# Meeso1/nmmo

Hardware: AMD Instinct MI355X
Metric: agent-steps/sec (whole node), 128-agent envs at 1/2/4/8 MI355X (higher is better)
Workload: dtype int16

## Files before the change

__graft_entry__.py:

```python

import os
import sys

ROOT = os.path.dirname(os.path.abspath(__file__))
if ROOT not in sys.path:
    sys.path.insert(0, ROOT)


def build() -> None:
    from nmmo_amd import build as nb

    nb.build(verbose=True)
    nb.build_heads(verbose=True)
    nb.build_ppo(verbose=True)
    nb.build_lstm(verbose=True)
    from oracle import oracle

    oracle.build(force=True)
    import nmmo_amd
    from nmmo_amd import _native

    _native.lib()
    from nmmo_amd import heads

    heads.lib()
    from nmmo_amd import ppo

    ppo.lib()
    from nmmo_amd import lstm

    lstm.lib()


def smoke() -> None:
    import numpy as np
    import torch

    from nmmo_amd.config import Config
    from nmmo_amd.engine import NmmoEngine
    from oracle.oracle import OracleEnvs

    assert torch.cuda.is_available(), "smoke() needs cuda:0"
    torch.cuda.set_device(0)
    cfg = Config.preset("C4", MAP_N=4, early_stop_agent_num=8)
    eng = NmmoEngine(cfg, 2, seed=3)
# ... 20 lines not shown
```

nmmo_amd/build.py:

```python

from __future__ import annotations

import concurrent.futures
import functools
import hashlib
import os
import subprocess
import sys
import tempfile
from typing import NamedTuple

HERE = os.path.dirname(os.path.abspath(__file__))
CSRC = os.path.join(HERE, "csrc")
INCLUDE = os.path.join(HERE, "..", "include")
LIB_DIR = os.path.join(HERE, "lib")
ARCH = os.environ.get("NMMO_OFFLOAD_ARCH", "gfx950")


class Lib(NamedTuple):
    file: str
    sources: list
    headers: list
    include: list
    link: list = []


LIBS = {
    "hip": Lib("libnmmo_hip.so",
               ["mapgen.hip", "tick.hip", "obs.hip", "wrap.hip", "storage.hip", "wire.hip", "wire_obs.hip",
                "native_obs.hip", "flat_obs.hip", "p2p.hip", "capi.hip"],
               ["agent_obs.h", "common.h", "host_api.h", "kernels.h", "obs_layout.h", "wire.h"], ["nmmo_hip.h"],
               ["-ldl"]),
    "heads": Lib("libnmmo_heads.so", ["heads.hip", "tile_enc.hip", "item_enc.hip"], ["common.h", "host_api.h"],
                 ["nmmo_hip.h", "nmmo_heads.h"]),
    "ppo": Lib("libnmmo_ppo.so", ["ppo.hip"], ["host_api.h"], ["nmmo_ppo.h"]),
    "lstm": Lib("libnmmo_lstm.so", ["lstm.hip"], ["host_api.h"], ["nmmo_lstm.h"]),
}
SOURCES, HEADERS = LIBS["hip"].sources, LIBS["hip"].headers
LIB_PATH = os.path.join(LIB_DIR, LIBS["hip"].file)
STAMPS_PATH = os.path.join(LIB_DIR, "libnmmo_hip_stamps.so")
FLAGS = [
    f"--offload-arch={ARCH}", "-O3", "-std=c++17", "-fPIC", "-fvisibility=hidden", "-Wall", "-Werror",
    "-ffp-contract=off",
]


def _hipcc() -> str:
    for cand in (os.environ.get("HIPCC"), "/opt/rocm/bin/hipcc", "hipcc"):
        if cand and (os.path.sep not in cand or os.path.exists(cand)):
            return cand
    raise RuntimeError("hipcc not found")


def lib_path(name: str = "hip") -> str:
    return os.path.join(LIB_DIR, LIBS[name].file)


def source_hash(name: str = "hip") -> str:
    row = LIBS[name]
    h = hashlib.sha256()
    for f in [os.path.join(CSRC, f) for f in row.sources + row.headers] + [
            os.path.join(INCLUDE, f) for f in row.include]:
        with open(f, "rb") as fh:
            h.update(os.path.basename(f).encode() + b"\0" + fh.read())
    return h.hexdigest()[:16]


def stale(name: str = "hip") -> bool:
    if not os.path.exists(lib_path(name)):
        return True
    with open(lib_path(name), "rb") as fh:
        return ("src=" + source_hash(name)).encode() not in fh.read()


def build_lib(name: str, force: bool = False, verbose: bool = False, stamps: bool = False) -> str:
    row = LIBS[name]
    if stamps and name != "hip":
        raise ValueError("only the product library has a stamps variant")
    out = STAMPS_PATH if stamps else lib_path(name)
    if not force and not stamps and not stale(name):
        return out
    os.makedirs(LIB_DIR, exist_ok=True)
    tmp = out + ".tmp"
    flags = [*FLAGS, *(["-DNMMO_STAMPS"] if stamps else []), f'-DNMMO_SRC_HASH="{source_hash(name)}"']
    with tempfile.TemporaryDirectory(prefix="nmmo_build_") as d:
        objs = [os.path.join(d, f + ".o") for f in row.sources]
        cmds = [[_hipcc(), *flags, "-c", os.path.join(CSRC, f), "-o", o] for f, o in zip(row.sources, objs)]
        if verbose:
            print("\n".join(" ".join(c) for c in cmds), file=sys.stderr)
        jobs = max(1, min(len(cmds), os.cpu_count() or 1, int(os.environ.get("MAX_JOBS", "8"))))
        with concurrent.futures.ThreadPoolExecutor(jobs) as ex:
            for f in [ex.submit(subprocess.check_call, c) for c in cmds]:
                f.result()
        subprocess.check_call([_hipcc(), f"--offload-arch={ARCH}", "-shared", "-fPIC", *objs, *row.link, "-o", tmp])
    os.replace(tmp, out)
    return out


build = functools.partial(build_lib, "hip")
build_heads = functools.partial(build_lib, "heads")
build_ppo = functools.partial(build_lib, "ppo")
build_lstm = functools.partial(build_lib, "lstm")


if __name__ == "__main__":
    for lib_name in LIBS:
        print(build_lib(lib_name, force="--force" in sys.argv, verbose=True))
```

nmmo_amd/csrc/agent_obs.h:

```cpp
#pragma once

#include <utility>

#include "kernels.h"
#include "wire.h"

namespace nmmo {

#ifndef NMMO_AO_WAVES
#define NMMO_AO_WAVES 4
#define NMMO_AO_AGENTS 16
#endif
constexpr int kAoWaves = NMMO_AO_WAVES;
constexpr int kAoAgents = NMMO_AO_AGENTS;
constexpr int kAoRows = kMaxSlots / 64;
constexpr uint32_t kAoEmpty = 0xFFFFFFFFu;
static_assert(kSize <= 256 && kMaxSlots <= 2 * 256 && kMaxSlots % 64 == 0, "packed entity word; two slots per thread (>= 256 threads)");
__host__ __device__ constexpr int ao_stride(int S) { return ((S + 1) >> 1 | 1) << 1; }
__host__ __device__ constexpr size_t ao_columns_lds(int S) {
  return ((size_t)NMMO_N_ENTITY_COLS * ao_stride(S) * 2 + 15) & ~(size_t)15;
}
constexpr size_t kAoPkBytes = (size_t)(kMaxSlots + 64) * 4;
__host__ __device__ constexpr size_t ao_entity_lds(int S) { return ao_columns_lds(S) + kAoPkBytes; }
__host__ __device__ inline uint32_t ao_pack(int slot, int row, int col, bool immune, bool danger, bool player) {
// ... 212 lines not shown
    const uint64_t b = __ballot(in);
    const int pos = nvis + __popcll(b & lanes_below());
    if (in && pos < kNObs) visw[pos] = x;
    nvis += __popcll(b);
  }
  return nvis;
}

__device__ __forceinline__ void ao_window_offsets(int (&mo)[2]) {
  mo[0] = mo[1] = 0;
#pragma unroll
  for (int i = 0; i < 4; i++) {
    const int t = lane_id() + 64 * i;
    const int o = t < 225 ? (t / 15 - kVision) * kSize + t % 15 - kVision : 0;
    mo[i >> 1] |= (o & 0xFFFF) << (16 * (i & 1));
  }
}
__device__ __forceinline__ int ao_window_off(const int (&mo)[2], int i) {
  return (int)(int16_t)(uint16_t)((uint32_t)mo[i >> 1] >> (16 * (i & 1)));
}

static_assert(F_ALCHEMY_LEVEL == F_MELEE_LEVEL + 14 && F_FISHING_LEVEL == F_MELEE_LEVEL + 6 &&
                  F_HERBALISM_LEVEL == F_MELEE_LEVEL + 8, "skill level fields");
__host__ __device__ constexpr uint64_t ao_req_lut() {
  uint64_t m = 0;
  for (int t = 0; t < 16; t++) {
    const int k = (t >= T_SPEAR && t <= T_WAND) ? t - T_SPEAR : (t >= T_WHETSTONE && t <= T_RUNES) ? t - T_WHETSTONE
                  : (t >= T_ROD && t <= T_CHISEL) ? 3 + t - T_ROD : 8;
    m |= (uint64_t)k << (4 * t);
  }
  return m;
}
static_assert(T_RATION == 16 && T_POTION == 17, "requirement table: ration -> fishing, potion -> herbalism");
__device__ __forceinline__ uint64_t ao_usable_ballot(const int16_t* T, int Sp, int ti, uint2 it, bool have) {
  const int lane = ao_lane();
  int lv = 0;
  if (lane < 8) {
    lv = T[(F_MELEE_LEVEL + 2 * lane) * Sp + ti];
  } else if (lane == 8) {
    lv = max((int)T[F_MELEE_LEVEL * Sp + ti], max((int)T[F_RANGE_LEVEL * Sp + ti], (int)T[F_MAGE_LEVEL * Sp + ti]));
  }
  const int type = it_type(it);
  const int k = type < 16 ? (int)((ao_req_lut() >> (4 * type)) & 15u) : type == T_RATION ? 3 : type == T_POTION ? 4 : 8;
  const int req = __shfl(lv, k);
  const bool eq = type >= T_HAT && type <= T_RUNES && it_equipped(it);
  return __ballot(have && !it_price(it) && (eq || it_level(it) <= req));
}

struct AoSections {
  uint64_t s0, s1[2], s3, s4, s5[2], s6[2], s7[2], s8, s9, s10[2], s11;
};
struct AoAgent {
  int a, ti, r, c, gold, aid, nv, ninv, prev_price;
  uint32_t mv;
};
template <bool kWrap>
__device__ __forceinline__ AoSections ao_sections(const ObsParams& p, const int16_t* T, int Sp, const uint32_t* visw,
                                                 const AoAgent& g, uint2 it) {
  const bool combat = (p.systems & NMMO_SYS_COMBAT) != 0;
  const bool item = (p.systems & NMMO_SYS_ITEM) != 0;
  const bool exch = item && (p.systems & NMMO_SYS_EXCHANGE) != 0;
  const bool no_give = kWrap && (p.wflags & kWrapObsNoGive);
  const bool no_danger = kWrap && (p.wflags & kWrapObsNoDangerous);
  const int lane = ao_lane();
  AoSections x;
  x.s1[0] = x.s1[1] = x.s5[0] = x.s5[1] = x.s7[0] = x.s7[1] = 0ull;
#pragma unroll
  for (int h = 0; h < 2; h++) {
    if (64 * h >= g.nv) break;
    const int k = 64 * h + lane;
    bool tgt = false, st = false;
    if (k < g.nv) {
      const uint32_t w = visw[k];
      const int q = ao_slot(w);
      tgt = combat && q != g.a && linf(g.r, g.c, ao_row(w), ao_col(w)) <= 3 && !ao_immune(w) &&
            !(no_danger && ao_danger(w));
      st = ao_player(w) && q != g.a && ao_row(w) == g.r && ao_col(w) == g.c;
    }
    x.s1[h] = __ballot(tgt);
    const uint64_t sb = __ballot(st);
    if (item && !no_give) x.s5[h] = sb;
    if (exch && !no_give) x.s7[h] = sb;
  }
  x.s1[1] |= 1ull << (kNObs - 64);
  x.s5[1] |= 1ull << (kNObs - 64);
  x.s7[1] |= 1ull << (kNObs - 64);
  const bool have = lane < g.ninv;
  const bool fr = have && !it_equipped(it) && !it_price(it);
  const uint64_t bfr = __ballot(fr);
  x.s3 = (item ? bfr : 0ull) | 1ull << kInv;
  x.s4 = (item && !no_give ? bfr : 0ull) | 1ull << kInv;
  x.s9 = (exch ? __ballot(have && !it_equipped(it)) : 0ull) | 1ull << kInv;
  x.s11 = (item ? ao_usable_ballot(T, Sp, g.ti, it, have) : 0ull) | 1ull << kInv;
  x.s0 = combat ? low_bits(kSecN[0]) : 0ull;
  x.s6[0] = x.s6[1] = x.s10[0] = x.s10[1] = 0ull;
  if (exch) {
    const int ng = no_give ? min(g.gold, 1) : min(g.gold, kSecN[6]);
    x.s6[0] = low_bits(ng);
    x.s6[1] = low_bits(ng - 64);
    x.s10[0] = low_bits(kSecN[10]);
    x.s10[1] = low_bits(kSecN[10] - 64);
    if constexpr (kWrap) {
      const int pp = g.prev_price;
      if ((p.wflags & kWrapObsPrice) && pp >= 0 && pp < kSecN[10]) {
        const uint64_t clr = ~(1ull << (pp & 63));
        if (pp < 64) x.s10[0] &= clr;
        else x.s10[1] &= clr;
      }
    }
  }
// ... 25 lines not shown
```

nmmo_amd/csrc/capi.hip:

```cpp
#include <math.h>
#include <stdlib.h>
#include <string.h>

#include <algorithm>
#include <map>
#include <mutex>
#include <vector>

#include "host_api.h"
#include "kernels.h"
#include "wire.h"

using namespace nmmo;

#define HIP_TRY(expr)                                                                    \
  do {                                                                                   \
    hipError_t _e = (expr);                                                              \
    if (_e != hipSuccess) return fail(NMMO_E_HIP, "%s: %s", #expr, hipGetErrorString(_e)); \
  } while (0)

struct NmmoHandle {
  NmmoConfig cfg;
  NmmoLayout layout;
  DevState st;
// ... 537 lines not shown
  if (fr && fr[0] == '1') HIP_TRY(hipMemAddressFree(ptr, a.bytes));
  return NMMO_OK;
}

int nmmo_set_step_records(NmmoHandle* h, uint8_t* dev_records, int32_t* dev_fault) {
  if (!h) return fail(NMMO_E_INVALID, "null handle");
  if (dev_records && h->cfg.obs_layout != NMMO_OBS_WIRE)
    return fail(NMMO_E_INVALID, "nmmo_set_step_records: step records come with the wire obs layout");
  if (dev_fault && !dev_records) return fail(NMMO_E_INVALID, "nmmo_set_step_records: dev_fault without records");
  h->d_recs = dev_records;
  h->d_recs_fault = dev_fault;
  return NMMO_OK;
}

int nmmo_obs_bind(NmmoHandle* h, const void* obs) {
  if (!h) return fail(NMMO_E_INVALID, "null handle");
  if (!h->d_zrow) return obs ? fail(NMMO_E_INVALID, "nmmo_obs_bind: flat or native obs layouts only") : NMMO_OK;
  HIP_TRY(hipSetDevice(h->device));
  HIP_TRY(hipDeviceSynchronize());
  HIP_TRY(hipMemset(h->d_zrow, 0, (size_t)h->st.n_envs * h->st.P * 8));
  h->zbuf = obs;
  h->ztag = obs ? h->ztag + 1 : h->ztag;
  return NMMO_OK;
}

int nmmo_obs_invalidate(NmmoHandle* h, void* stream) {
  if (!h) return fail(NMMO_E_INVALID, "null handle");
  if (!h->d_zrow) return NMMO_OK;
  HIP_TRY(hipSetDevice(h->device));
  HIP_TRY(hipMemsetAsync(h->d_zrow, 0, (size_t)h->st.n_envs * h->st.P * 8, (hipStream_t)stream));
  return NMMO_OK;
}

__global__ void obs_forget_envs_kernel(uint64_t* zrow, const int32_t* ids, int n_ids, int n_envs, int P) {
  const int i = blockIdx.x, e = ids[i];
  if ((unsigned)e >= (unsigned)n_envs) return;
  for (int a = threadIdx.x; a < P; a += blockDim.x) zrow[(size_t)e * P + a] = 0;
}

int nmmo_obs_invalidate_envs(NmmoHandle* h, const int32_t* env_ids, int32_t n_ids, void* stream) {
  if (!h) return fail(NMMO_E_INVALID, "null handle");
  if (n_ids < 0 || n_ids > h->st.n_envs) return fail(NMMO_E_INVALID, "n_ids %d not in 0..%d", n_ids, h->st.n_envs);
  if (n_ids > 0 && !env_ids) return fail(NMMO_E_INVALID, "null env_ids");
  if (!h->d_zrow || n_ids == 0) return NMMO_OK;
  HIP_TRY(hipSetDevice(h->device));
  hipLaunchKernelGGL(obs_forget_envs_kernel, dim3(n_ids), dim3(128), 0, (hipStream_t)stream, h->d_zrow, env_ids,
                     n_ids, h->st.n_envs, h->st.P);
  HIP_TRY(hipGetLastError());
  return NMMO_OK;
}

__global__ void obs_forget_tile_kernel(uint64_t* zst, const int32_t* ids, int n_envs, int P) {
  const int e = ids ? ids[blockIdx.x] : (int)blockIdx.x;
  if ((unsigned)e >= (unsigned)n_envs) return;
  for (int a = threadIdx.x; a < P; a += blockDim.x) zst[(size_t)e * P + a] |= kZsTile;
}

int nmmo_obs_invalidate_sections(NmmoHandle* h, const int32_t* env_ids, int32_t n_ids, uint32_t sections,
                                 void* stream) {
  if (!h) return fail(NMMO_E_INVALID, "null handle");
  if (!env_ids) n_ids = h->st.n_envs;
  if (n_ids < 0 || n_ids > h->st.n_envs) return fail(NMMO_E_INVALID, "n_ids %d not in 0..%d", n_ids, h->st.n_envs);
  if (!h->d_zrow || n_ids == 0 || sections == 0) return NMMO_OK;
  HIP_TRY(hipSetDevice(h->device));
  const bool tile_only = sections == NMMO_OBS_SEC_TILE && h->cfg.obs_layout == NMMO_OBS_FLAT;
  if (!tile_only) {
// ... 682 lines not shown
```

nmmo_amd/csrc/flat_obs.hip:

```cpp
#include "agent_obs.h"

namespace nmmo {

#ifndef NMMO_FO_ABL
#define NMMO_FO_ABL 0
#endif
#ifndef NMMO_FO_STAMPS
#define NMMO_FO_STAMPS 0
#endif
#if NMMO_FO_STAMPS
constexpr int kFoStamps = 12;
__device__ uint64_t fo_stamp_buf[1 << 17][kFoStamps];
__device__ uint64_t fo_wave_buf[1 << 15][6];
#define FO_STAMP(k) fst[k] = __builtin_amdgcn_s_memtime()
#else
#define FO_STAMP(k) (void)0
#endif
#ifndef NMMO_FO_XCD
#define NMMO_FO_XCD 1
#endif
#ifndef NMMO_FO_TILE_SKIP
#define NMMO_FO_TILE_SKIP 0
#endif
#ifndef NMMO_FO_TASK_BATCH
// ... 86 lines not shown
  return (uint64_t)(uint32_t)__builtin_amdgcn_readlane((int)g.lo, g.j10 + slot) |
         (uint64_t)(uint32_t)__builtin_amdgcn_readlane((int)g.hi, g.j10 + slot) << 32;
}
template <int kC>
__device__ __forceinline__ void fo_put(float* row, FoImg& g, uint64_t m, float aid, float tick) {
  constexpr int sl = fo_slot(kC);
  const int lane = ao_lane();
  const bool same = g.ext && m == fo_prev(g, sl);
  if constexpr (kC == kFoChunks - 1) {
    constexpr int n = kMaskN - 64 * kC;
    if (!same) {
      if (lane < n + 2) fo_st(row, 64 * kC + lane, lane < n ? fo_bit(m) : lane == n ? aid : tick);
      g.nst += n + 2;
    } else {
      if (lane == n + 1) fo_st(row, 64 * kC + lane, tick);
      g.nst += 1;
    }
  } else if (!same) {
    fo_st(row, 64 * kC + lane, fo_bit(m));
    g.nst += 64;
  }
  g.nimg = writelane<2 * sl>((int)(uint32_t)m, g.nimg);
  g.nimg = writelane<2 * sl + 1>((int)(uint32_t)(m >> 32), g.nimg);
}
template <int kC>
__device__ __forceinline__ void fo_tail_chunks(float* row, FoImg& g, const AoSections& x, uint64_t buy17, float aid,
                                               float tick) {
  if constexpr (kC < kFoChunks) {
    uint64_t m = fo_chunk<kC>(x);
    if constexpr (kC == kFoTail0) m |= buy17 | 1ull << ((kWireBuyLo + NMMO_MARKET_ROWS) & 63);
    fo_put<kC>(row, g, m, aid, tick);
    fo_tail_chunks<kC + 1>(row, g, x, buy17, aid, tick);
  }
}

struct IcDesc {
  uint32_t tmA, tmB;
  uint32_t f;
};
__device__ __forceinline__ IcDesc ic_desc(int col) {
  auto bits = [](int lo, int hi) { return ((2u << hi) - 1u) & ~((1u << lo) - 1u); };
  IcDesc d{0u, 0u, 0u};
  auto bf = [&](int sel, int sh, int wd) { d.f = (uint32_t)(sel | sh << 1 | wd << 6); };
  switch (col) {
    case 0: bf(1, 16, 16); break;
    case 1: bf(0, 0, 5); break;
    case 2: d.f = 1u << 11; break;
    case 3: bf(0, 5, 4); break;
    case 5: bf(1, 0, 16); break;
    case 6: case 7: case 8:
      d.tmA = 1u << (T_SPEAR + col - 6) | 1u << (T_WHETSTONE + col - 6);
      d.f = 5u << 12 | 5u << 20;
      break;
    case 9: case 10: case 11:
      d.tmA = bits(T_HAT, T_BOTTOM);
      d.tmB = bits(T_ROD, T_CHISEL);
      d.f = 3u << 12 | 2u << 16;
      break;
    case 12: d.tmA = 1u << T_POTION; d.f = 5u << 12 | 50u << 20; break;
    case 13: d.tmA = 1u << T_RATION; d.f = 5u << 12 | 50u << 20; break;
    case 14: bf(0, 9, 1); break;
    case 15: bf(0, 10, 7); break;
    default: break;
  }
  return d;
}
// ... 162 lines not shown
  const int nm = min(max(sg.nm, 0), NMMO_MARKET_ROWS), nst = fo_staged(nm);
  const uint2 lwd = ao_listing_load(p, e, sg);
  auto listings = [&]() {
    if constexpr (kMirror) {
      uint4* gd = reinterpret_cast<uint4*>(gat) + w * kGatIt * 64 + lane;
      gd[0] = gq0;
      if constexpr (kGatIt > 1) gd[64] = gq1;
      if constexpr (kGatIt > 2) gd[128] = gq2;
      if constexpr (kGatIt > 3) gd[192] = gq3;
    }
    if (tid < nm) {
      mpo[tid] = (uint16_t)(it_price(lwd) | ((sg.mv >> 16) & 255) << 8);
      if (tid < nst) mtop[-tid] = lwd;
    }
    for (int j = tid + (int)blockDim.x; j < nm; j += blockDim.x) {
      const int v = p.mlist[(size_t)e * NMMO_MARKET_ROWS + j];
      const int own = (v >> 16) & 255, slot = (v >> 24) & 15;
      const uint2 wd = p.items[((size_t)e * P + own) * kInv + slot];
      mpo[j] = (uint16_t)(it_price(wd) | own << 8);
      if (j < nst) mtop[-j] = wd;
    }
  };
  if constexpr (kMirror)
    ao_stage_windows_at<kAoAgents, kFoWinRowBytes / 4, true>(p, e, g, wpr, wpc, wst, ist, listings);
  else
    ao_stage_windows<kAoAgents, kFoWinRowBytes / 4>(p, e, g, T, Sp, wst, ist, listings, []() { __syncthreads(); });
#if NMMO_FO_STAMPS
  wst_[2] = __builtin_amdgcn_s_memtime();
#endif
  asm volatile("" : "+v"(img.x), "+v"(img.y), "+v"(pinv.x), "+v"(pinv.y), "+v"(my_prev));
  if (!img_ok) img = make_uint2(0u, 0u);
  if (!pinv_ok) pinv = make_uint2(0u, 0u);
  const int my_h = !zvl ? (kNObs | NMMO_MARKET_ROWS << 12) : zzl ? 0 : (zs_hv(my_s) | zs_hm(my_s) << 12);
  int nrows = 0;
  unsigned long long nbytes = 0;
  int wo[2];
  ao_win_offsets<kFoWinRowBytes>(wo);
  int toff[4];
#pragma unroll
  for (int i = 0; i < 4; i++) {
    const int t = lane + 64 * i;
    toff[i] = ((t / 15 - kVision) & 255) | (t % 15 - kVision) * 256;
  }
  const int ef = lane & 31, eh = lane >> 5;
  const int iq = lane >> 4;
  const IcDesc icd = ic_desc(lane & 15);

#if NMMO_FO_STAMPS
  wst_[3] = __builtin_amdgcn_s_memtime();
#endif
#pragma unroll 1
  for (int j = 0; j < ((NMMO_FO_ABL & 64) ? 0 : kPerWave); j++) {
    const int a = abase + kAoWaves * j;
    if (a >= P) break;
    const int lane = ao_lane();
    FoArgs kp = (FoArgs)__builtin_amdgcn_kernarg_segment_ptr();
    asm volatile("" : "+s"(kp));
    auto grow = (__attribute__((address_space(1))) float*)(p.obs + ((NMMO_FO_ABL & 256)
        ? (size_t)(((e * P + a) & 15) + 16 * (blockIdx.x & 7)) : (size_t)e * P + a) * elems);
    asm volatile("" : "+s"(grow));
    float* row = (float*)grow;
    const bool zv = (zvalid >> j) & 1;
    const int hj = __builtin_amdgcn_readlane(my_h, j);
    const int hv = hj & 4095, hm = hj >> 12;
    if (!__builtin_amdgcn_readlane(my_alive, j)) {
      if ((zzero >> j) & 1) {
// ... 8 lines not shown
      if (zv) {
        wave_zero(row, 0, kFlatEntity + hv * NMMO_N_ENTITY_COLS);
        wave_zero(row, kFlatInv, kFlatMarket + hm * 16);
        wave_zero(row, kFlatTask, elems);
        nbytes += 4ull * (kFlatEntity + hv * NMMO_N_ENTITY_COLS + kFlatMarket + hm * 16 - kFlatInv + elems - kFlatTask);
      } else {
        wave_zero(row, 0, elems);
        nbytes += 4ull * elems;
      }
      if (lane == 0) {
        kp->zrow[(size_t)e * P + a] = kp->ztag;
        kp->zst[(size_t)e * P + a] = kZsZero;
      }
      nrows++;
      continue;
    }
    nrows++;
#if NMMO_FO_STAMPS
    uint64_t fst[kFoStamps];
#endif
    FO_STAMP(0);
    const int la = a - g * kAoAgents;
    const int rcj = __builtin_amdgcn_readlane((int)my_rc, j);
    const int r = (int16_t)(rcj & 0xFFFF), c = rcj >> 16;
    const int16_t* Ta = kMirror ? T + la * kMirrorCols : T;
    const int Spa = kMirror ? 1 : Sp, tia = kMirror ? 0 : a;
    if constexpr (kMirror) visw = visw_all + (w * kPerWave + j) * kFoVisw;
    const int gold = __builtin_amdgcn_readfirstlane(Ta[F_GOLD * Spa + tia]);
    const int aid = __builtin_amdgcn_readfirstlane(Ta[F_ID * Spa + tia]);
    const uint8_t* wa = wsb + la * kFoWinAgentBytes;
    uint32_t wm[4];
#pragma unroll
    for (int i = 0; i < 4; i++) wm[i] = lane + 64 * i < 225 ? wa[ao_win_off(wo, i)] : 0u;
    const uint2 it = lane < kInv ? ist[la * kInv + lane] : make_uint2(0u, 0u);
    const uint32_t mv = ao_move_bits(wm[1]);
    const int ninv = __builtin_ctzll(~__ballot(lane < kInv && it_type(it) != 0));
    int nv;
    if constexpr (kMirror) {
      nv = __builtin_amdgcn_readlane(my_nv, j);
    } else {
      nv = (NMMO_FO_ABL & 32) ? 0 : min(fo_compact(pr, r, c, visw), kNObs);
      __builtin_amdgcn_fence(__ATOMIC_RELEASE, "wavefront");
      __builtin_amdgcn_wave_barrier();
      __builtin_amdgcn_fence(__ATOMIC_ACQUIRE, "wavefront");
    }

    FO_STAMP(1);
    const bool ext = (zextv >> j) & 1;
    FoImg fg{ext, img.x, img.y, 10 * j, 0, 0};
    if (!(NMMO_FO_ABL & 1)) {
      AoAgent ag;
      ag.a = a;
      ag.ti = tia;
      ag.r = r;
      ag.c = c;
      ag.gold = gold;
      ag.aid = aid;
      ag.nv = nv;
      ag.ninv = ninv;
      ag.prev_price = kWrap ? __builtin_amdgcn_readlane(my_prev, j) : -1;
      ag.mv = mv;
      const AoSections x = ao_sections<kWrap>(p, Ta, Spa, visw, ag, it);
      FO_STAMP(2);
      fg.ext = ext;
      fo_put<0>(row, fg, fo_chunk<0>(x), 0.f, 0.f);
      auto buy_word = [&](int m) {
        const int k = 64 * m + lane;
        bool bv = false;
        if (exch && k < nm) {
          const uint32_t po = mpo[k];
          bv = (int)(po & 255u) <= gold && (int)(po >> 8) != a;
        }
        return __ballot(bv);
      };
      const int nbuy = max(nm, hm);
      const int clast = max(1, min((kWireBuyLo + nbuy - 1) >> 6, 16));
      uint64_t bprev = nm > 0 ? buy_word(0) : 0ull;
      fo_put<1>(row, fg, fo_chunk<1>(x) | bprev << (kWireBuyLo & 63), 0.f, 0.f);
      FO_STAMP(3);
#pragma unroll 1
      for (int cc = 2; cc <= clast; cc++) {
        const uint64_t bcur = 64 * (cc - 1) < nm ? buy_word(cc - 1) : 0ull;
        fo_st(row, 64 * cc + lane, fo_bit(bcur << (kWireBuyLo & 63) | bprev >> (64 - (kWireBuyLo & 63))));
// ... 18 lines not shown
        if (ef < NMMO_N_ENTITY_COLS) {
          float v = 0.f;
          if (k < nv) {
            const uint32_t vw = visw[k];
            const int tv = kMirror ? gj[k * kMirrorCols + ef] : T[ef * Sp + ao_slot(vw)];
            v = (float)(epos ? (int)((vw >> esh) & 255u) : tv);
          }
          fo_st(row, de + k0 * NMMO_N_ENTITY_COLS, v);
        }
      }
      if constexpr (kMirror) {
        if (nv2 > kFoGather) {
          const int16_t* Mk = kp->frows + (size_t)e * kMaxSlots * kMirrorCols;
#pragma unroll 1
          for (int k0 = kFoGather; k0 < nv2; k0 += 2) {
            const int k = k0 + eh;
            if (ef < NMMO_N_ENTITY_COLS) {
              float v = 0.f;
              if (k < nv) {
                const uint32_t vw = visw[k];
                const int tv = Mk[(size_t)min(ao_slot(vw), kMaxSlots - 1) * kMirrorCols + ef];
                v = (float)(epos ? (int)((vw >> esh) & 255u) : tv);
              }
              fo_st(row, de + k0 * NMMO_N_ENTITY_COLS, v);
            }
          }
        }
      }
      const int hz = max(nv2, hv);
      wave_zero(row, kFlatEntity + nv2 * NMMO_N_ENTITY_COLS, kFlatEntity + hz * NMMO_N_ENTITY_COLS);
      nbytes += 4ull * (hz * NMMO_N_ENTITY_COLS + max(nm, hm) * 16);
    }
    FO_STAMP(6);
    const int jl = (12 * j + lane) & 63;
    const uint32_t px = (uint32_t)__shfl((int)pinv.x, jl), py = (uint32_t)__shfl((int)pinv.y, jl);
    const bool inv_same = ext && __ballot(lane < kInv && (px != it.x || py != it.y)) == 0ull;
    if (!inv_same) {
#pragma unroll
      for (int h = 0; h < ((NMMO_FO_ABL & 4) ? 0 : kInv * 16 / 64); h++) {
        const int q = 4 * h + iq;
        float v = 0.f;
        if (4 * h < ninv && q < ninv) v = ic_value(ist[la * kInv + q], aid, icd);
        fo_st(row, kFlatInv + 64 * h + lane, v);
      }
      nbytes += 4ull * kInv * 16;
    }
    FO_STAMP(7);
    const int nms = (NMMO_FO_ABL & 8) ? 0 : fo_staged(nm);
    for (int k = lane; k < nms * 16; k += 64) fo_st(row, kFlatMarket + k, ic_value(mtop[-(k >> 4)], (mpo[k >> 4] >> 8) + 1, icd));
    if (nm > nms && !(NMMO_FO_ABL & 8)) {
      for (int k = nms * 16 + lane; k < nm * 16; k += 64) {
        const int q = k >> 4;
        const int v = kp->mlist[(size_t)e * NMMO_MARKET_ROWS + q];
        const uint2 wd = kp->items[((size_t)e * P + ((v >> 16) & 255)) * kInv + ((v >> 24) & 15)];
        fo_st(row, kFlatMarket + k, ic_value(wd, (mpo[q] >> 8) + 1, icd));
      }
    }
    wave_zero(row, kFlatMarket + nm * 16, kFlatMarket + max(nm, hm) * 16);
    FO_STAMP(8);
    const int task = __builtin_amdgcn_readlane(my_task, j);
    if (!((ztask >> j) & 1)) {
      const float* temb = kp->task + (size_t)task * tdim;
      int k0 = 0;
      for (; k0 + kFoTaskBatch * 64 <= tdim; k0 += kFoTaskBatch * 64) {
        float t[kFoTaskBatch];
#pragma unroll
        for (int i = 0; i < kFoTaskBatch; i++) t[i] = temb[k0 + 64 * i + lane];
#pragma unroll
        for (int i = 0; i < kFoTaskBatch; i++) fo_st(row, kFlatTask + k0 + 64 * i + lane, t[i]);
      }
      for (int k = k0 + lane; k < tdim; k += 64) fo_st(row, kFlatTask + k, temb[k]);
      nbytes += 4ull * tdim;
    }
    FO_STAMP(9);
    const uint32_t ppos = (uint32_t)__builtin_amdgcn_readlane((int)img.x, 40 + j);
    const bool tkn = NMMO_FO_TILE_SKIP && ext && !((ztile >> j) & 1);
    const bool same_r = tkn && (int)(ppos & 255u) == r, same_c = tkn && (int)((ppos >> 8) & 255u) == c;
    if (!(NMMO_FO_ABL & 16)) {
      float* dt = row + kFlatTask + tdim + 3 * lane;
#pragma unroll
      for (int i = 0; i < 4; i++) {
        if (lane + 64 * i < 225) {
          const float vr = (float)(r + ((toff[i] << 24) >> 24)), vc = (float)(c + (toff[i] >> 8)), vm = (float)wm[i];
          if (NMMO_FO_TILE_SKIP) {
            if (!same_r) dt[192 * i] = vr;
            if (!same_c) dt[192 * i + 1] = vc;
            dt[192 * i + 2] = vm;
          } else {
            typedef float f3 __attribute__((ext_vector_type(3)));
            const f3 v = {vr, vc, vm};
            __builtin_memcpy(dt + 192 * i, &v, 12);
          }
        }
      }
      nbytes += 4ull * 225 * (1 + !same_r + !same_c);
    }
    FO_STAMP(10);
    {
      uint32_t* zx = reinterpret_cast<uint32_t*>(kp->zext + ((size_t)e * P + a) * kZext);
      int wv = fg.nimg;
      if (lane == 20) wv = r | c << 8;
      if (lane == 21) wv = 0;
      if (lane < 22) zx[lane] = (uint32_t)wv;
      if (!inv_same && lane < kInv) reinterpret_cast<uint2*>(zx + 22)[lane] = it;
      if (lane == 0) {
        if (!zv) kp->zrow[(size_t)e * P + a] = kp->ztag;
        kp->zst[(size_t)e * P + a] = zs_pack(nv2, nm, task) | kZsExt;
      }
    }
#if NMMO_FO_STAMPS
    FO_STAMP(11);
    if (lane == 0 && (size_t)e * P + a < (1u << 17))
      for (int k = 0; k < kFoStamps; k++) fo_stamp_buf[(size_t)e * P + a][k] = fst[k];
#endif
    if constexpr (!kMirror) {
      __builtin_amdgcn_fence(__ATOMIC_RELEASE, "wavefront");
      __builtin_amdgcn_wave_barrier();
      __builtin_amdgcn_fence(__ATOMIC_ACQUIRE, "wavefront");
    }
  }
#if NMMO_FO_STAMPS
  wst_[4] = __builtin_amdgcn_s_memtime();
  wst_[5] = (uint64_t)e | (uint64_t)nrows << 32;
  {
    const size_t wi = ((size_t)blockIdx.y * gridDim.x + blockIdx.x) * kAoWaves + w;
    if (lane == 0 && wi < (1u << 15))
      for (int k = 0; k < 6; k++) fo_wave_buf[wi][k] = wst_[k];
  }
#endif
  if (p.rows_out && lane == 0 && nrows) {
    atomicAdd(&p.rows_out[2 * e], (unsigned long long)nrows);
// ... 52 lines not shown
```

nmmo_amd/engine.py:

```python

from __future__ import annotations

import ctypes

import numpy as np
import torch

from . import abi
from ._native import NativeError, check, layout, lib


class TickFault(NativeError):

    def __init__(self, word: int, where: str = ""):
        self.word = int(word)
        self.code, self.env = self.word & 0xFF, self.word >> 8
        what = abi.FAULT_NAMES.get(self.code, f"code {self.code}")
        super().__init__(f"{where + ': ' if where else ''}tick fault word {self.word:#x}: {what} "
                         f"(env / list position {self.env})")


class NmmoEngine:
    def __init__(self, config, n_envs: int, seed: int = 0, device=None, task_embedding=None,
                 env_index_base: int = 0):
# ... 197 lines not shown
    def set_step_records(self, records, fault=None):
        if records is not None and (records.dtype != torch.uint8 or records.device != self.device
                                    or not records.is_contiguous() or records.numel() < 8 * self.n_envs * self.P):
            raise ValueError("records must be a contiguous uint8 tensor of >= 8 * n_envs * P bytes on the "
                             "engine's device")
        if fault is not None and (fault.dtype != torch.int32 or fault.device != self.device):
            raise ValueError("fault must be an int32 tensor on the engine's device")
        self._step_records = (records, fault)
        check(lib().nmmo_set_step_records(self.h, None if records is None else ctypes.c_void_p(records.data_ptr()),
                                          None if fault is None else ctypes.c_void_p(fault.data_ptr())),
              "nmmo_set_step_records")

    def obs_invalidate(self):
        check(lib().nmmo_obs_invalidate(self.h, self._stream()), "nmmo_obs_invalidate")

    def obs_invalidate_envs(self, env_ids):
        if env_ids.dtype != torch.int32 or env_ids.device != self.device or not env_ids.is_contiguous():
            raise ValueError("env_ids must be a contiguous int32 tensor on the engine's device")
        with torch.cuda.device(self.device):
            check(lib().nmmo_obs_invalidate_envs(self.h, self._ptr(env_ids), env_ids.numel(), self._stream()),
                  "nmmo_obs_invalidate_envs")
        self._inv_ids = env_ids

    def obs_invalidate_sections(self, sections: int, env_ids=None):
        if env_ids is not None and (env_ids.dtype != torch.int32 or env_ids.device != self.device
                                    or not env_ids.is_contiguous()):
            raise ValueError("env_ids must be a contiguous int32 tensor on the engine's device")
        with torch.cuda.device(self.device):
            check(lib().nmmo_obs_invalidate_sections(self.h, None if env_ids is None else self._ptr(env_ids),
                                                     0 if env_ids is None else env_ids.numel(), int(sections),
                                                     self._stream()), "nmmo_obs_invalidate_sections")
        self._inv_ids = env_ids

    def get_fault(self) -> int:
        f = ctypes.c_int32()
        check(lib().nmmo_get_fault(self.h, ctypes.byref(f)), "nmmo_get_fault")
        return f.value

    def check_fault(self, where: str = ""):
        f = self.get_fault()
        if f:
            raise TickFault(f, where)

    def fault_into(self, dst):
        with torch.cuda.device(self.device):
            check(lib().nmmo_fault_into(self.h, self._ptr(dst), self._stream()), "nmmo_fault_into")

    def inject_fault(self, word: int):
        check(lib().nmmo_inject_fault(self.h, int(word)), "nmmo_inject_fault")

    def read_timing(self):
        ms = (ctypes.c_double * 3)()
        n = ctypes.c_int32()
        check(lib().nmmo_read_timing(self.h, ms, ctypes.byref(n)), "nmmo_read_timing")
        return ms[0], ms[1], n.value, ms[2]

    def get_state(self) -> np.ndarray:
        n = self.layout.state_bytes_per_env * self.n_envs
        buf = np.zeros(n, np.uint8)
        check(lib().nmmo_get_state(self.h, buf.ctypes.data_as(ctypes.c_void_p), n), "nmmo_get_state")
        return buf

    def set_state(self, buf: np.ndarray):
        buf = np.ascontiguousarray(buf, dtype=np.uint8)
        check(lib().nmmo_set_state(self.h, buf.ctypes.data_as(ctypes.c_void_p), buf.nbytes),
              "nmmo_set_state")
# ... 55 lines not shown
```

Measured before the change: 328.1 million.

## Batch action-mask computation across a wave's agents in mirror flat-obs path

Adds a per-wave mask pass that computes the action-mask chunks, buy-order ballots, inventory diffs and zext row state for all agents in a wave at once, using 16-lane groups per agent instead of a full wave per agent. The per-agent loop then only stores the chunks that changed, read from the precomputed words, and skips its own inventory, move and zext bookkeeping in the mirror path. It also adds a test-hook library build and a debug API to read obs row state. This aims to cut the serial per-agent ballot and shuffle work and redundant loads, at the cost of more register pressure and more complex logic.

New measurement: 342.5 million, median of 6. 1.04x the previous value.

```diff
diff --git a/__graft_entry__.py b/__graft_entry__.py
--- a/__graft_entry__.py
+++ b/__graft_entry__.py
@@ -11,6 +11,7 @@
     from nmmo_amd import build as nb
 
     nb.build(verbose=True)
+    nb.build_hooks(verbose=True)
     nb.build_heads(verbose=True)
     nb.build_ppo(verbose=True)
     nb.build_lstm(verbose=True)
diff --git a/nmmo_amd/build.py b/nmmo_amd/build.py
--- a/nmmo_amd/build.py
+++ b/nmmo_amd/build.py
@@ -39,6 +39,7 @@
 SOURCES, HEADERS = LIBS["hip"].sources, LIBS["hip"].headers
 LIB_PATH = os.path.join(LIB_DIR, LIBS["hip"].file)
 STAMPS_PATH = os.path.join(LIB_DIR, "libnmmo_hip_stamps.so")
+HOOKS_PATH = os.path.join(LIB_DIR, "libnmmo_hip_hooks.so")
 FLAGS = [
     f"--offload-arch={ARCH}", "-O3", "-std=c++17", "-fPIC", "-fvisibility=hidden", "-Wall", "-Werror",
     "-ffp-contract=off",
@@ -73,16 +74,25 @@
         return ("src=" + source_hash(name)).encode() not in fh.read()
 
 
-def build_lib(name: str, force: bool = False, verbose: bool = False, stamps: bool = False) -> str:
+def _embeds(path: str, name: str) -> bool:
+    if not os.path.exists(path):
+        return False
+    with open(path, "rb") as fh:
+        return ("src=" + source_hash(name)).encode() in fh.read()
+
+
+def build_lib(name: str, force: bool = False, verbose: bool = False, stamps: bool = False, hooks: bool = False) -> str:
     row = LIBS[name]
-    if stamps and name != "hip":
-        raise ValueError("only the product library has a stamps variant")
-    out = STAMPS_PATH if stamps else lib_path(name)
-    if not force and not stamps and not stale(name):
+    if (stamps or hooks) and name != "hip":
+        raise ValueError("only the product library has variants")
+    out = STAMPS_PATH if stamps else HOOKS_PATH if hooks else lib_path(name)
+    if not force and hooks and _embeds(out, name):
+        return out
+    if not force and not stamps and not hooks and not stale(name):
         return out
     os.makedirs(LIB_DIR, exist_ok=True)
     tmp = out + ".tmp"
-    flags = [*FLAGS, *(["-DNMMO_STAMPS"] if stamps else []), f'-DNMMO_SRC_HASH="{source_hash(name)}"']
+    flags = [*FLAGS, *(["-DNMMO_STAMPS"] if stamps else []), *(["-DNMMO_TEST_HOOKS"] if hooks else []), f'-DNMMO_SRC_HASH="{source_hash(name)}"']
     with tempfile.TemporaryDirectory(prefix="nmmo_build_") as d:
         objs = [os.path.join(d, f + ".o") for f in row.sources]
         cmds = [[_hipcc(), *flags, "-c", os.path.join(CSRC, f), "-o", o] for f, o in zip(row.sources, objs)]
@@ -98,6 +108,7 @@
 
 
 build = functools.partial(build_lib, "hip")
+build_hooks = functools.partial(build_lib, "hip", hooks=True)
 build_heads = functools.partial(build_lib, "heads")
 build_ppo = functools.partial(build_lib, "ppo")
 build_lstm = functools.partial(build_lib, "lstm")
@@ -106,3 +117,4 @@
 if __name__ == "__main__":
     for lib_name in LIBS:
         print(build_lib(lib_name, force="--force" in sys.argv, verbose=True))
+    print(build_hooks(force="--force" in sys.argv, verbose=True))
diff --git a/nmmo_amd/csrc/agent_obs.h b/nmmo_amd/csrc/agent_obs.h
--- a/nmmo_amd/csrc/agent_obs.h
+++ b/nmmo_amd/csrc/agent_obs.h
@@ -268,6 +268,14 @@
   return m;
 }
 static_assert(T_RATION == 16 && T_POTION == 17, "requirement table: ration -> fishing, potion -> herbalism");
+__device__ __forceinline__ int ao_req_lane(int type) {
+  return type < 16 ? (int)((ao_req_lut() >> (4 * type)) & 15u) : type == T_RATION ? 3 : type == T_POTION ? 4 : 8;
+}
+__device__ __forceinline__ bool ao_usable(uint2 it, bool have, int req) {
+  const int type = it_type(it);
+  const bool eq = type >= T_HAT && type <= T_RUNES && it_equipped(it);
+  return have && !it_price(it) && (eq || it_level(it) <= req);
+}
 __device__ __forceinline__ uint64_t ao_usable_ballot(const int16_t* T, int Sp, int ti, uint2 it, bool have) {
   const int lane = ao_lane();
   int lv = 0;
@@ -276,11 +284,15 @@
   } else if (lane == 8) {
     lv = max((int)T[F_MELEE_LEVEL * Sp + ti], max((int)T[F_RANGE_LEVEL * Sp + ti], (int)T[F_MAGE_LEVEL * Sp + ti]));
   }
-  const int type = it_type(it);
-  const int k = type < 16 ? (int)((ao_req_lut() >> (4 * type)) & 15u) : type == T_RATION ? 3 : type == T_POTION ? 4 : 8;
-  const int req = __shfl(lv, k);
-  const bool eq = type >= T_HAT && type <= T_RUNES && it_equipped(it);
-  return __ballot(have && !it_price(it) && (eq || it_level(it) <= req));
+  const int req = __shfl(lv, ao_req_lane(it_type(it)));
+  return __ballot(ao_usable(it, have, req));
+}
+
+__device__ __forceinline__ void ao_row_preds(uint32_t w, int a, int r, int c, bool combat, bool no_danger, bool& tgt,
+                                             bool& st) {
+  const int q = ao_slot(w);
+  tgt = combat && q != a && linf(r, c, ao_row(w), ao_col(w)) <= 3 && !ao_immune(w) && !(no_danger && ao_danger(w));
+  st = ao_player(w) && q != a && ao_row(w) == r && ao_col(w) == c;
 }
 
 struct AoSections {
@@ -307,11 +319,7 @@
     const int k = 64 * h + lane;
     bool tgt = false, st = false;
     if (k < g.nv) {
-      const uint32_t w = visw[k];
-      const int q = ao_slot(w);
-      tgt = combat && q != g.a && linf(g.r, g.c, ao_row(w), ao_col(w)) <= 3 && !ao_immune(w) &&
-            !(no_danger && ao_danger(w));
-      st = ao_player(w) && q != g.a && ao_row(w) == g.r && ao_col(w) == g.c;
+      ao_row_preds(visw[k], g.a, g.r, g.c, combat, no_danger, tgt, st);
     }
     x.s1[h] = __ballot(tgt);
     const uint64_t sb = __ballot(st);
diff --git a/nmmo_amd/csrc/capi.hip b/nmmo_amd/csrc/capi.hip
--- a/nmmo_amd/csrc/capi.hip
+++ b/nmmo_amd/csrc/capi.hip
@@ -593,6 +593,22 @@
   return NMMO_OK;
 }
 
+#ifdef NMMO_TEST_HOOKS
+__attribute__((visibility("default"))) int nmmo_debug_obs_row_state(NmmoHandle* h, uint64_t* tag, uint64_t* zrow,
+                                                                     uint64_t* zst, uint64_t* zext) {
+  if (!h || !tag || !zrow || !zst || !zext) return fail(NMMO_E_INVALID, "null argument");
+  if (!h->d_zrow || !h->d_zext) return fail(NMMO_E_INVALID, "nmmo_debug_obs_row_state: flat obs layout only");
+  const size_t rows = (size_t)h->st.n_envs * h->st.P;
+  HIP_TRY(hipSetDevice(h->device));
+  HIP_TRY(hipDeviceSynchronize());
+  HIP_TRY(hipMemcpy(zrow, h->d_zrow, rows * 8, hipMemcpyDeviceToHost));
+  HIP_TRY(hipMemcpy(zst, h->d_zrow + rows, rows * 8, hipMemcpyDeviceToHost));
+  HIP_TRY(hipMemcpy(zext, h->d_zext, rows * kZext * 8, hipMemcpyDeviceToHost));
+  *tag = h->zbuf ? h->ztag : 0;
+  return NMMO_OK;
+}
+#endif
+
 __global__ void obs_forget_envs_kernel(uint64_t* zrow, const int32_t* ids, int n_ids, int n_envs, int P) {
   const int i = blockIdx.x, e = ids[i];
   if ((unsigned)e >= (unsigned)n_envs) return;
diff --git a/nmmo_amd/csrc/flat_obs.hip b/nmmo_amd/csrc/flat_obs.hip
--- a/nmmo_amd/csrc/flat_obs.hip
+++ b/nmmo_amd/csrc/flat_obs.hip
@@ -142,6 +142,166 @@
     fo_put<kC>(row, g, m, aid, tick);
     fo_tail_chunks<kC + 1>(row, g, x, buy17, aid, tick);
   }
+}
+
+constexpr int kFoPassRows = 16;
+static_assert(kFoPassRows == 16 && kAoAgents / kAoWaves * kFoPassRows <= 64 && kInv <= kFoPassRows &&
+                  kFoGather <= kFoPassRows, "a 16-lane group per agent");
+constexpr int kFoBuyLane = 48;
+struct FoPass {
+  uint32_t lo, hi;
+  uint64_t chg;
+  uint64_t idiff;
+};
+template <int kSl>
+__device__ __forceinline__ void fo_pass_chunks(const AoSections& x, int sl, uint64_t& m) {
+  if constexpr (kSl < 10) {
+    constexpr int c = kSl < 2 ? kSl : kSl - 2 + kFoTail0;
+    static_assert(fo_slot(c) == kSl, "tracked chunk");
+    const uint64_t mc = fo_chunk<c>(x);
+    if (sl == kSl) m = mc;
+    fo_pass_chunks<kSl + 1>(x, sl, m);
+  }
+}
+template <bool kWrap>
+__device__ __forceinline__ FoPass fo_mask_pass(const ObsParams& p, int e, int w, int abase, int nm, const int16_t* own,
+                                               const uint32_t* visw, const uint8_t* wsb, const uint2* ist,
+                                               const uint16_t* mpo, int my_nv, uint32_t my_rc, int my_prev, int my_alive,
+                                               int my_task, uint64_t zvalid, uint64_t zextv, uint2 img, uint2 pinv) {
+  constexpr int kPerWave = kAoAgents / kAoWaves;
+  const bool combat = (p.systems & NMMO_SYS_COMBAT) != 0;
+  const bool item = (p.systems & NMMO_SYS_ITEM) != 0;
+  const bool exch = item && (p.systems & NMMO_SYS_EXCHANGE) != 0;
+  const bool no_give = kWrap && (p.wflags & kWrapObsNoGive);
+  const bool no_danger = kWrap && (p.wflags & kWrapObsNoDangerous);
+  const int lane = lane_id(), P = p.P;
+  const int gj = lane >> 4, gk = lane & 15, ga = abase + kAoWaves * gj, gla = w + kAoWaves * gj;
+  const int grc = __shfl((int)my_rc, gj);
+  const int gr = (int16_t)(grc & 0xFFFF), gc = grc >> 16;
+  bool tgt = false, st = false;
+  if (gk < __shfl(my_nv, gj)) ao_row_preds(visw[gj * kFoVisw + gk], ga, gr, gc, combat, no_danger, tgt, st);
+  const uint64_t tb = __ballot(tgt), sb = __ballot(st);
+  const uint2 it = gk < kInv ? ist[gla * kInv + gk] : make_uint2(0u, 0u);
+  const uint64_t occ = __ballot(gk < kInv && it_type(it) != 0);
+  const bool have = gk < __builtin_ctz(~((uint32_t)(occ >> (16 * gj)) & 0xFFFFu));
+  const uint64_t bfr = __ballot(have && !it_equipped(it) && !it_price(it));
+  const uint64_t bse = __ballot(have && !it_equipped(it));
+  uint64_t bus;
+  {
+    const int16_t* lvs = own + gla * kMirrorCols + F_MELEE_LEVEL;
+    int lv = 0;
+    if (gk < 8) lv = lvs[2 * gk];
+    else if (gk == 8) lv = max((int)lvs[0], max((int)lvs[F_RANGE_LEVEL - F_MELEE_LEVEL], (int)lvs[F_MAGE_LEVEL - F_MELEE_LEVEL]));
+    const int req = __shfl(lv, 16 * gj + ao_req_lane(it_type(it)));
+    bus = __ballot(ao_usable(it, have, req));
+  }
+  const int ja = min(lane / 10, kPerWave - 1), sl = lane - 10 * (lane / 10), la = w + kAoWaves * ja;
+  const uint64_t noop = 1ull << (kNObs - 64);
+  uint64_t t0 = (uint32_t)(tb >> (16 * ja)) & 0xFFFFu, t1 = 0ull, s0 = (uint32_t)(sb >> (16 * ja)) & 0xFFFFu, s1 = 0ull;
+#pragma unroll 1
+  for (int j = 0; j < kPerWave; j++) {
+    const int nv = __builtin_amdgcn_readlane(my_nv, j);
+    if (nv <= kFoPassRows) continue;
+    const int rcj = __builtin_amdgcn_readlane((int)my_rc, j), a = abase + kAoWaves * j;
+    const int r = (int16_t)(rcj & 0xFFFF), c = rcj >> 16;
+    uint64_t tj[2] = {0ull, 0ull}, sj[2] = {0ull, 0ull};
+#pragma unroll
+    for (int h = 0; h < 2; h++) {
+      if (64 * h >= nv) break;
+      const int k = 64 * h + lane;
+      bool tg = false, sm = false;
+      if (k < nv) ao_row_preds(visw[j * kFoVisw + k], a, r, c, combat, no_danger, tg, sm);
+      tj[h] = __ballot(tg);
+      sj[h] = __ballot(sm);
+    }
+    if (ja == j) t0 = tj[0], t1 = tj[1], s0 = sj[0], s1 = sj[1];
+  }
+  AoSections x;
+  x.s1[0] = t0;
+  x.s1[1] = t1 | noop;
+  x.s5[0] = item && !no_give ? s0 : 0ull;
+  x.s5[1] = (item && !no_give ? s1 : 0ull) | noop;
+  x.s7[0] = exch && !no_give ? s0 : 0ull;
+  x.s7[1] = (exch && !no_give ? s1 : 0ull) | noop;
+  const uint64_t ifr = (uint32_t)(bfr >> (16 * ja)) & 0xFFFFu;
+  x.s3 = (item ? ifr : 0ull) | 1ull << kInv;
+  x.s4 = (item && !no_give ? ifr : 0ull) | 1ull << kInv;
+  x.s9 = (exch ? (uint64_t)((uint32_t)(bse >> (16 * ja)) & 0xFFFFu) : 0ull) | 1ull << kInv;
+  x.s11 = (item ? (uint64_t)((uint32_t)(bus >> (16 * ja)) & 0xFFFFu) : 0ull) | 1ull << kInv;
+  x.s0 = combat ? low_bits(kSecN[0]) : 0ull;
+  x.s6[0] = x.s6[1] = x.s10[0] = x.s10[1] = 0ull;
+  if (exch) {
+    const int gold = own[la * kMirrorCols + F_GOLD];
+    const int ng = no_give ? min(gold, 1) : min(gold, kSecN[6]);
+    x.s6[0] = low_bits(ng);
+    x.s6[1] = low_bits(ng - 64);
+    x.s10[0] = low_bits(kSecN[10]);
+    x.s10[1] = low_bits(kSecN[10] - 64);
+    if constexpr (kWrap) {
+      const int pp = __shfl(my_prev, ja);
+      if ((p.wflags & kWrapObsPrice) && pp >= 0 && pp < kSecN[10]) {
+        const uint64_t clr = ~(1ull << (pp & 63));
+        if (pp < 64) x.s10[0] &= clr;
+        else x.s10[1] &= clr;
+      }
+    }
+  }
+  {
+    const uint8_t* wa = wsb + la * kFoWinAgentBytes;
+    uint32_t b = 0u;
+#pragma unroll
+    for (int d = 0; d < 5; d++)
+      if (!impassable((int)wa[(kVision + dir_dr(d)) * kFoWinRowBytes + kVision + dir_dc(d)])) b |= 1u << d;
+    x.s8 = b;
+  }
+  uint64_t m = 0ull;
+  fo_pass_chunks<0>(x, sl, m);
+  uint64_t bw0 = 0ull, bw15 = 0ull;
+  FoPass o;
+  o.lo = img.x;
+  o.hi = img.y;
+  if (exch && nm > 0) {
+    const uint32_t po0 = lane < nm ? mpo[lane] : 0u, po15 = 15 * 64 + lane < nm ? mpo[15 * 64 + lane] : 0u;
+#pragma unroll
+    for (int j = 0; j < kPerWave; j++) {
+      const int a = abase + kAoWaves * j;
+      const int gold = __builtin_amdgcn_readfirstlane((int)own[(w + kAoWaves * j) * kMirrorCols + F_GOLD]);
+      const uint64_t b0 = __ballot(lane < nm && (int)(po0 & 255u) <= gold && (int)(po0 >> 8) != a);
+      uint64_t b15 = 0ull;
+      if (nm > 15 * 64) b15 = __ballot(15 * 64 + lane < nm && (int)(po15 & 255u) <= gold && (int)(po15 >> 8) != a);
+      if (ja == j) bw0 = b0, bw15 = b15;
+      if (lane == kFoBuyLane + j) o.lo = (uint32_t)b0, o.hi = (uint32_t)(b0 >> 32);
+    }
+  }
+  if (sl == 1) m |= bw0 << (kWireBuyLo & 63);
+  if (sl == 2) m |= bw15 >> (64 - (kWireBuyLo & 63)) | 1ull << ((kWireBuyLo + NMMO_MARKET_ROWS) & 63);
+  const bool ext = (zextv >> ja) & 1;
+  o.chg = __ballot(lane < 10 * kPerWave && (!ext || (uint32_t)m != img.x || (uint32_t)(m >> 32) != img.y));
+  if (lane < 10 * kPerWave) o.lo = (uint32_t)m, o.hi = (uint32_t)(m >> 32);
+  const int ji = min(lane / kInv, kPerWave - 1);
+  const uint2 iw = ist[(w + kAoWaves * ji) * kInv + lane % kInv];
+  const bool idl = lane < kInv * kPerWave && (!((zextv >> ji) & 1) || iw.x != pinv.x || iw.y != pinv.y);
+  o.idiff = __ballot(idl);
+  {
+    const int jp = lane < 10 * kPerWave ? ja : min(lane - 10 * kPerWave, kPerWave - 1);
+    const size_t ai = (size_t)e * P + min(abase + kAoWaves * jp, P - 1);
+    uint2 wv = make_uint2(o.lo, o.hi);
+    const int rcp = __shfl((int)my_rc, jp);
+    if (lane >= 10 * kPerWave) {
+      wv = make_uint2((uint32_t)((int)(int16_t)(rcp & 0xFFFF) | (rcp >> 16) << 8), 0u);
+    }
+    const int alp = __shfl(my_alive, jp);
+    if (lane < 11 * kPerWave && alp) reinterpret_cast<uint2*>(p.zext)[ai * kZext + (lane < 10 * kPerWave ? sl : 10)] = wv;
+    const size_t ii = (size_t)e * P + min(abase + kAoWaves * ji, P - 1);
+    const int ali = __shfl(my_alive, ji);
+    if (idl && ali) reinterpret_cast<uint2*>(p.zext)[ii * kZext + 11 + lane % kInv] = iw;
+    if (lane < kPerWave && my_alive) {
+      const size_t am = (size_t)e * P + abase + kAoWaves * lane;
+      if (!((zvalid >> lane) & 1)) p.zrow[am] = p.ztag;
+      p.zst[am] = zs_pack((my_nv + 1) & ~1, nm, my_task) | kZsExt;
+    }
+  }
+  return o;
 }
 
 struct IcDesc {
@@ -370,6 +530,12 @@
   if (!img_ok) img = make_uint2(0u, 0u);
   if (!pinv_ok) pinv = make_uint2(0u, 0u);
   const int my_h = !zvl ? (kNObs | NMMO_MARKET_ROWS << 12) : zzl ? 0 : (zs_hv(my_s) | zs_hm(my_s) << 12);
+  FoPass mp{img.x, img.y, ~0ull, ~0ull};
+  if constexpr (kMirror) {
+    if (!(NMMO_FO_ABL & 1))
+      mp = fo_mask_pass<kWrap>(p, e, w, abase, nm, T, visw, wsb, ist, mpo, my_nv, my_rc, my_prev, my_alive, my_task, zvalid,
+                               zextv, img, pinv);
+  }
   int nrows = 0;
   unsigned long long nbytes = 0;
   int wo[2];
@@ -444,9 +610,14 @@
     uint32_t wm[4];
 #pragma unroll
     for (int i = 0; i < 4; i++) wm[i] = lane + 64 * i < 225 ? wa[ao_win_off(wo, i)] : 0u;
-    const uint2 it = lane < kInv ? ist[la * kInv + lane] : make_uint2(0u, 0u);
-    const uint32_t mv = ao_move_bits(wm[1]);
-    const int ninv = __builtin_ctzll(~__ballot(lane < kInv && it_type(it) != 0));
+    uint2 it = make_uint2(0u, 0u);
+    uint32_t mv = 0u;
+    int ninv = 0;
+    if constexpr (!kMirror) {
+      it = lane < kInv ? ist[la * kInv + lane] : make_uint2(0u, 0u);
+      mv = ao_move_bits(wm[1]);
+      ninv = __builtin_ctzll(~__ballot(lane < kInv && it_type(it) != 0));
+    }
     int nv;
     if constexpr (kMirror) {
       nv = __builtin_amdgcn_readlane(my_nv, j);
@@ -460,7 +631,58 @@
     FO_STAMP(1);
     const bool ext = (zextv >> j) & 1;
     FoImg fg{ext, img.x, img.y, 10 * j, 0, 0};
-    if (!(NMMO_FO_ABL & 1)) {
+    if constexpr (kMirror) {
+      if (!(NMMO_FO_ABL & 1)) {
+        const uint32_t chg = (uint32_t)(mp.chg >> (10 * j)) & 0x3FFu;
+        auto pm = [&](int l) {
+          return (uint64_t)(uint32_t)__builtin_amdgcn_readlane((int)mp.lo, l) |
+                 (uint64_t)(uint32_t)__builtin_amdgcn_readlane((int)mp.hi, l) << 32;
+        };
+        int nst = 0;
+        FO_STAMP(2);
+#pragma unroll 1
+        for (uint32_t cs = chg & 3u; cs; cs &= cs - 1u) {
+          const int s = __builtin_ctz(cs);
+          fo_st(row, 64 * s + lane, fo_bit(pm(10 * j + s)));
+          nst += 64;
+        }
+        FO_STAMP(3);
+        auto buy_word = [&](int m) {
+          const int k = 64 * m + lane;
+          bool bv = false;
+          if (exch && k < nm) {
+            const uint32_t po = mpo[k];
+            bv = (int)(po & 255u) <= gold && (int)(po >> 8) != a;
+          }
+          return __ballot(bv);
+        };
+        const int clast = max(1, min((kWireBuyLo + max(nm, hm) - 1) >> 6, 16));
+        uint64_t bprev = pm(kFoBuyLane + j);
+#pragma unroll 1
+        for (int cc = 2; cc <= clast; cc++) {
+          const uint64_t bcur = 64 * (cc - 1) < nm ? buy_word(cc - 1) : 0ull;
+          fo_st(row, 64 * cc + lane, fo_bit(bcur << (kWireBuyLo & 63) | bprev >> (64 - (kWireBuyLo & 63))));
+          bprev = bcur;
+        }
+        FO_STAMP(4);
+#pragma unroll 1
+        for (uint32_t cs = (chg >> 2) & 0x7Fu; cs; cs &= cs - 1u) {
+          const int s = __builtin_ctz(cs);
+          fo_st(row, 64 * (kFoTail0 + s) + lane, fo_bit(pm(10 * j + 2 + s)));
+          nst += 64;
+        }
+        constexpr int kc = kFoChunks - 1, n = kMaskN - 64 * kc;
+        if (chg >> 9) {
+          const uint64_t m = pm(10 * j + 9);
+          if (lane < n + 2) fo_st(row, 64 * kc + lane, lane < n ? fo_bit(m) : lane == n ? (float)aid : tickf);
+          nst += n + 2;
+        } else {
+          if (lane == n + 1) fo_st(row, 64 * kc + lane, tickf);
+          nst += 1;
+        }
+        nbytes += 4ull * (nst + 64 * (clast - 1));
+      }
+    } else if (!(NMMO_FO_ABL & 1)) {
       AoAgent ag;
       ag.a = a;
       ag.ti = tia;
@@ -545,10 +767,16 @@
       nbytes += 4ull * (hz * NMMO_N_ENTITY_COLS + max(nm, hm) * 16);
     }
     FO_STAMP(6);
-    const int jl = (12 * j + lane) & 63;
-    const uint32_t px = (uint32_t)__shfl((int)pinv.x, jl), py = (uint32_t)__shfl((int)pinv.y, jl);
-    const bool inv_same = ext && __ballot(lane < kInv && (px != it.x || py != it.y)) == 0ull;
+    bool inv_same;
+    if constexpr (kMirror) {
+      inv_same = ((uint32_t)(mp.idiff >> (kInv * j)) & ((1u << kInv) - 1u)) == 0u;
+    } else {
+      const int jl = (12 * j + lane) & 63;
+      const uint32_t px = (uint32_t)__shfl((int)pinv.x, jl), py = (uint32_t)__shfl((int)pinv.y, jl);
+      inv_same = ext && __ballot(lane < kInv && (px != it.x || py != it.y)) == 0ull;
+    }
     if (!inv_same) {
+      if constexpr (kMirror) ninv = __builtin_ctzll(~__ballot(lane < kInv && it_type(ist[la * kInv + min(lane, kInv - 1)]) != 0));
 #pragma unroll
       for (int h = 0; h < ((NMMO_FO_ABL & 4) ? 0 : kInv * 16 / 64); h++) {
         const int q = 4 * h + iq;
@@ -586,7 +814,7 @@
       nbytes += 4ull * tdim;
     }
     FO_STAMP(9);
-    const uint32_t ppos = (uint32_t)__builtin_amdgcn_readlane((int)img.x, 40 + j);
+    const uint32_t ppos = (uint32_t)__builtin_amdgcn_readlane((int)(kMirror ? mp.lo : img.x), 40 + j);
     const bool tkn = NMMO_FO_TILE_SKIP && ext && !((ztile >> j) & 1);
     const bool same_r = tkn && (int)(ppos & 255u) == r, same_c = tkn && (int)((ppos >> 8) & 255u) == c;
     if (!(NMMO_FO_ABL & 16)) {
@@ -609,7 +837,7 @@
       nbytes += 4ull * 225 * (1 + !same_r + !same_c);
     }
     FO_STAMP(10);
-    {
+    if constexpr (!kMirror) {
       uint32_t* zx = reinterpret_cast<uint32_t*>(kp->zext + ((size_t)e * P + a) * kZext);
       int wv = fg.nimg;
       if (lane == 20) wv = r | c << 8;
diff --git a/nmmo_amd/engine.py b/nmmo_amd/engine.py
--- a/nmmo_amd/engine.py
+++ b/nmmo_amd/engine.py
@@ -253,6 +253,18 @@
                                                      self._stream()), "nmmo_obs_invalidate_sections")
         self._inv_ids = env_ids
 
+    def obs_row_state(self):
+        f = getattr(lib(), "nmmo_debug_obs_row_state", None)
+        if f is None:
+            raise NativeError("obs_row_state needs the hook build of the library (build.build_hooks, NMMO_LIB)")
+        f.argtypes, f.restype = [ctypes.c_void_p] * 5, ctypes.c_int
+        n, P = self.n_envs, self.P
+        tag = ctypes.c_uint64()
+        zrow, zst, zext = (np.zeros(s, np.uint64) for s in ((n, P), (n, P), (n, P, 23)))
+        with torch.cuda.device(self.device):
+            check(f(self.h, ctypes.byref(tag), zrow.ctypes.data, zst.ctypes.data, zext.ctypes.data), "nmmo_debug_obs_row_state")
+        return (zrow == np.uint64(tag.value)) & (tag.value != 0), zst, zext
+
     def get_fault(self) -> int:
         f = ctypes.c_int32()
         check(lib().nmmo_get_fault(self.h, ctypes.byref(f)), "nmmo_get_fault")
```
